# briandaniel/ParallelNonlinearOptimizationLibrary

Hardware: AMD Instinct MI355X
Metric: LM iters/sec at m=16384,n=2048 (higher is better)
Workload: dtype f64

## Files before the change

### parallelnonlinearoptimizationlibrary_amd/csrc/kernels/blas.hip

```cpp
#include "../pnol_internal.hpp"
#include "../pnol_comm.hpp"
#include "../pnol_env.hpp"

#include <cstdlib>

namespace pnol {
namespace {

constexpr int kWave = 64;

__device__ __forceinline__ double wave_sum(double v) {
#pragma unroll
    for (int m = 32; m >= 1; m >>= 1) v += __shfl_xor(v, m, kWave);
    return v;
}

constexpr int kU = 4;

template <int R>
__device__ __forceinline__ void gemv_load(double2 (&a)[R][kU], double2 (&xr)[kU], const double2* const (&arow)[R],
                                          const double2* __restrict__ xv, int base, int lane) {
#pragma unroll
    for (int u = 0; u < kU; ++u) xr[u] = xv[base + u * kWave + lane];
#pragma unroll
// ... 173 lines not shown
    __syncthreads();
    if (threadIdx.x < R && row0 + threadIdx.x < rows) {
        const int r = threadIdx.x;
        y[row0 + r] = -((part[0][r] + part[1][r]) + (part[2][r] + part[3][r]));
    }
}

template <int R, bool NT>
__global__ __launch_bounds__(256) void k_gemv_neg_wg(const double* __restrict__ A, long lda, int rows, int cols,
                                                     const double* __restrict__ x, double* __restrict__ y) {
    gemv_neg_wg_body<R, NT>(A, lda, rows, cols, x, y);
}

template <int R, bool VEC, bool XV>
__global__ __launch_bounds__(256) void k_gemv_neg_slices(const double* __restrict__ A, long lda, long sstride, int rows,
                                                         int m, int mS, int s0, const double* __restrict__ x,
                                                         double* __restrict__ y) {
    const int s = s0 + blockIdx.y;
    const int cols = max(0, min(mS, m - s * mS));
    gemv_neg_wg_body<R, true, VEC, XV>(A + (long)s * sstride, lda, rows, cols, x + (long)s * mS,
                                       y + (long)blockIdx.y * rows);
}

__global__ __launch_bounds__(256) void k_gemv_neg_scalar(const double* __restrict__ A, long lda, int rows, int cols,
                                                         const double* __restrict__ x, double* __restrict__ y) {
    const int lane = threadIdx.x & 63;
    const long row = (long)blockIdx.x * 4 + (threadIdx.x >> 6);
    if (row >= rows) return;
    const double* a = A + row * lda;
    double acc[4] = {0.0, 0.0, 0.0, 0.0};
    int c = lane;
    for (; c + 3 * kWave < cols; c += 4 * kWave)
// ... 302 lines not shown
#undef PNOL_GEMV_WG
        return launch_check();
    }
    int R = forced == 1 || forced == 2 || forced == 4 ? forced : (rows >= 8192 ? 2 : 1);
    const int blocks = (rows + 4 * R - 1) / (4 * R);
    if (R == 4)
        hipLaunchKernelGGL((k_gemv_neg<4>), dim3(blocks), dim3(256), 0, ctx->stream, A, (long)lda, rows, cols, x, y);
    else if (R == 2)
        hipLaunchKernelGGL((k_gemv_neg<2>), dim3(blocks), dim3(256), 0, ctx->stream, A, (long)lda, rows, cols, x, y);
    else
        hipLaunchKernelGGL((k_gemv_neg<1>), dim3(blocks), dim3(256), 0, ctx->stream, A, (long)lda, rows, cols, x, y);
    return launch_check();
}

int launch_gemv_neg_slices(pnol_ctx* ctx, const double* A, int lda, long sstride, int rows, int m, int mS, int s0,
                           int nsl, const double* x, double* y, hipStream_t stream) {
    if (!stream) stream = ctx->stream;
    if (!A || !x || !y || rows <= 0 || nsl <= 0 || (mS & 1)) return PNOL_ERR_ARG;
    static const int R = [] {
        const int v = env_atoi("PNOL_JTR_ROWS", 2);
        return (v == 1 || v == 4) ? v : 2;
    }();
    const bool vec = !((lda & 1) || (sstride & 1) || !aligned16(A));
    const bool xvec = aligned16(x);
    const dim3 grid((rows + R - 1) / R, nsl);
#define PNOL_SLICES(RR, V, XV)                                                                                      \
    hipLaunchKernelGGL((k_gemv_neg_slices<RR, V, XV>), grid, dim3(256), 0, stream, A, (long)lda, sstride, rows, m, mS, \
                       s0, x, y)
#define PNOL_SLICES_R(V, XV) \
    do { if (R == 1) PNOL_SLICES(1, V, XV); else if (R == 4) PNOL_SLICES(4, V, XV); else PNOL_SLICES(2, V, XV); } while (0)
    if (vec && xvec) PNOL_SLICES_R(true, true);
    else if (xvec) PNOL_SLICES_R(false, true);
    else if (vec) PNOL_SLICES_R(true, false);
    else PNOL_SLICES_R(false, false);
#undef PNOL_SLICES_R
#undef PNOL_SLICES
    return launch_check();
}

int launch_gemv_neg_seq(pnol_ctx* ctx, const double* A, int lda, int rows, int cols, const double* x, double* y) {
    if (!A || !x || !y || rows <= 0 || cols <= 0 || lda < cols) return PNOL_ERR_ARG;
    int blocks = (rows + 63) / 64;
    hipLaunchKernelGGL(k_gemv_neg_seq, dim3(blocks), dim3(64), 0, ctx->stream, A, (long)lda, rows, cols, x, y);
// ... 128 lines not shown
```

### parallelnonlinearoptimizationlibrary_amd/csrc/kernels/chol.hip

```cpp
#include "../pnol_internal.hpp"
#include "../pnol_comm.hpp"
#include "../chol_tasks.hpp"
#include "../pnol_env.hpp"

#include <algorithm>
#include <cstdlib>
#include <type_traits>

namespace pnol {
namespace {

constexpr int NB = 64;
constexpr int kPad = 18;
constexpr int kSub = NB * kPad;
constexpr int kStage = 4 * kSub;
constexpr int kSpin = 1 << 24;
constexpr int kInfoTimeout = kCholTimeout;
typedef double d4 __attribute__((ext_vector_type(4)));

__device__ __forceinline__ double readlane_d(double v, int lane) {
    const int lo = __builtin_amdgcn_readlane(__double2loint(v), lane);
    const int hi = __builtin_amdgcn_readlane(__double2hiint(v), lane);
    return __hiloint2double(hi, lo);
}
// ... 1802 lines not shown
    CholWs w;
    const bool persist = chol_persistent(variant) && (n + NB - 1) / NB >= 2;
    PNOL_CHECK(chol_ws(ctx, n, persist, w));
    const int T = w.T, N = w.N;
    for (int k = -1; k <= (persist ? -1 : T - 2); ++k) {
        const int R = T - 1 - k;
        const int grid = k < 0 ? 2 + std::min(N, 1024) : R + R * (R + 1) / 2;
        const int epoch = ++ctx->chol4_epoch;
        hipLaunchKernelGGL(k_chol_step, dim3(grid), dim3(256), 0, ctx->stream, w.P, w.Lm, w.ldp, T, k, w.W, w.bv, w.zv,
                           w.rowflag, epoch, dinfo, A, (long)lda, n, rhs, w.pf, persist ? w.npf : 0);
    }
    if (persist) PNOL_CHECK(chol_persist_launch(ctx, ctx->stream, w, dinfo, RedArgs{}));
    return chol_bwd_launch(ctx, ctx->stream, w, n, sigma, dinfo, xbase, xnext, xnext != nullptr);
}

__global__ __launch_bounds__(256) void k_chol_reducing_prep(double* __restrict__ P, long ldp, int T, int n,
                                                            double* __restrict__ bv, int* __restrict__ pflags,
                                                            int npflags, int* __restrict__ info, int vinit,
                                                            int* __restrict__ zc, int nz) {
    const int N = T * NB, tid = blockIdx.x * blockDim.x + threadIdx.x, nth = gridDim.x * blockDim.x;
    const int b0 = 2 * T, v1 = 3 * T + T * T;
    for (int q = tid; q < npflags; q += nth) pflags[q] = (q >= b0 && q < v1) ? vinit : 0;
    for (int q = tid; q < nz; q += nth) zc[q] = 0;
    for (int r = n + tid; r < N; r += nth) bv[r] = 0.0;
    if (n < N) {
        const long pad = (long)(N - n) * N + (long)n * (N - n);
        for (long e = tid; e < pad; e += nth) {
            int r, c;
            if (e < (long)(N - n) * N) {
                r = n + (int)(e / N);
                c = (int)(e % N);
            } else {
                const long f = e - (long)(N - n) * N;
                r = (int)(f / (N - n));
                c = n + (int)(f % (N - n));
            }
            P[(long)r * ldp + c] = r == c ? 1.0 : 0.0;
        }
    }
    if (tid == 0) *info = 0;
}

int launch_chol_reducing_prep(pnol_ctx* ctx, int n, int* dinfo, CholRed& cr) {
    if (!dinfo || n <= NB) return PNOL_ERR_ARG;
    cr.n = n;
    cr.dinfo = dinfo;
    return chol_ws(ctx, n, true, cr.w);
}

int launch_chol_reducing_start(pnol_ctx* ctx, const CholRed& cr, bool preloaded, int* zc, int nz) {
    const CholWs& w = cr.w;
    const int n = cr.n;
    const long pad = (long)(w.N - n) * w.N + (long)n * (w.N - n), work = std::max<long>(pad, w.npf);
    hipLaunchKernelGGL(k_chol_reducing_prep, dim3((unsigned)std::max<long>(1, std::min<long>(1024, (work + 255) / 256))),
                       dim3(256), 0, ctx->stream, w.P, w.ldp, w.T, n, w.bv, w.pf, w.npf, cr.dinfo, preloaded ? 0 : -1,
                       zc, zc ? nz : 0);
    return launch_check();
}

static int chol_red_run(pnol_ctx* ctx, hipStream_t st, const CholRed& cr, const RedArgs& red, double* sigma,
                        const double* xbase, double* xnext) {
    PNOL_CHECK(chol_persist_launch(ctx, st, cr.w, cr.dinfo, red));
    return chol_bwd_launch(ctx, st, cr.w, cr.n, sigma, cr.dinfo, xbase, xnext, true);
}

int launch_chol_preloaded_run(pnol_ctx* ctx, hipStream_t st, const CholRed& cr, double* sigma, const double* xbase,
                              double* xnext) {
    if (!sigma) return PNOL_ERR_ARG;
    RedArgs red;
    red.n = cr.n;
    red.preloaded = true;
// ... 33 lines not shown
```

### parallelnonlinearoptimizationlibrary_amd/csrc/kernels/syrk.hip

```cpp
#include "../pnol_internal.hpp"
#include "../pnol_comm.hpp"
#include "../pnol_env.hpp"

#include <algorithm>
#include <type_traits>
#include <vector>

namespace pnol {
namespace {

typedef double d4 __attribute__((ext_vector_type(4)));

constexpr int kPad = 18;

__device__ __forceinline__ unsigned diag_blocks(int w) {
    constexpr unsigned T[8] = {
        56u | 57u << 6 | 58u << 12 | 59u << 18 | 60u << 24 | 1u << 30,
        48u | 49u << 6 | 50u << 12 | 51u << 18 | 52u << 24 | 1u << 30,
        40u | 41u << 6 | 42u << 12 | 43u << 18 | 44u << 24 | 1u << 30,
        32u | 33u << 6 | 34u << 12 | 35u << 18 | 36u << 24 | 1u << 30,
        61u | 62u << 6 | 63u << 12 | 0u << 18,
        53u | 54u << 6 | 8u << 12 | 9u << 18,
        45u | 16u << 6 | 17u << 12 | 18u << 18,
        24u | 25u << 6 | 26u << 12 | 27u << 18};
// ... 52 lines not shown
#pragma unroll
    for (int q = 0; q < NV; ++q) *reinterpret_cast<double2*>(dst + 2 * q) = s.v[q];
}

#ifdef PNOL_SYRK_TIMELINE
__device__ unsigned long long g_syrk_tl[3 * 65536];
#endif

template <bool NTS, bool SC1 = false>
__device__ __forceinline__ void part_store(double v, double* p) {
    if constexpr (SC1) __hip_atomic_store(p, v, __ATOMIC_RELAXED, __HIP_MEMORY_SCOPE_AGENT);
    else if constexpr (NTS) __builtin_nontemporal_store(v, p);
    else *p = v;
}

template <int MODE, int TILE, int NW = 4, bool NTS = true, bool SC1 = false, bool DLAST = false>
__device__ __forceinline__ int syrk_tile_body(const double* __restrict__ X, long ldx, int nr, int K, int split_k,
                                              int kfirst, int kchunk, int sub, int slice0, int mS, long sstride,
                                              double* __restrict__ part, int tile0, int bid, int nblk,
                                              double (&lds)[2][2][TILE * kPad]) {
    constexpr int NT = 64 * NW, WC = NW / 2;
    constexpr int WTM = TILE / 2, WTN = TILE / WC, NBM = WTM / 16, NBN = WTN / 16;
#ifdef PNOL_SYRK_TIMELINE
    const unsigned long long tl0 = __builtin_amdgcn_s_memrealtime();
#endif
    int blk, t, sidx;
    {
        const int ntl = nblk / split_k, nsl = split_k / sub;
        const int u0 = bid / (ntl * nsl), rest = bid % (ntl * nsl);
        int tl = rest / nsl;
        if (DLAST) {
            const int nt = (int)((sqrt(8.0 * ntl + 1.0) - 1.0) * 0.5 + 0.5);
            const int noff = ntl - nt;
            if (tl < noff) {
                int r = (int)((sqrt(8.0 * tl + 1.0) + 1.0) * 0.5);
                while (r * (r - 1) / 2 > tl) --r;
                while ((r + 1) * r / 2 <= tl) ++r;
                tl = r * (r + 1) / 2 + (tl - r * (r - 1) / 2);
            } else {
                const int d = tl - noff;
                tl = d * (d + 1) / 2 + d;
            }
        }
        sidx = (rest % nsl) * sub + u0;
        blk = tl * split_k + sidx;
        t = tile0 + tl;
    }
    int ti, tj;
    tile_of(t, ti, tj);
    const bool diag = ti == tj;
    const int prow0 = ti * TILE, qrow0 = tj * TILE;
    const int slice = slice0 + sidx / sub, u = sidx % sub;
    X += (long)slice * (sstride - mS);
    const int kbeg = slice * mS + (u == 0 ? 0 : kfirst + (u - 1) * kchunk);
    const int kend = min(K, min((slice + 1) * mS, u == 0 ? slice * mS + kfirst : kbeg + kchunk));
    const int nstages = kend > kbeg ? (kend - kbeg + kTK - 1) / kTK : 0;

    const int lane = threadIdx.x & 63;
    const int wave = threadIdx.x >> 6;
    const int wr = wave / WC, wc = wave % WC;
    const bool ldx_even = (ldx & 1) == 0;

// ... 124 lines not shown
#pragma unroll
                for (int ni = 0; ni < NBN; ++ni)
#pragma unroll
                    for (int r = 0; r < 4; ++r) {
                        int row = wr * WTM + mi * 16 + orow + 4 * r;
                        int col = wc * WTN + ni * 16 + ocol;
                        part_store<NTS, SC1>(acc[mi][ni][r], out + row * ld + col);
                    }
        }
    }
#ifdef PNOL_SYRK_TIMELINE
    if (threadIdx.x == 0) {
        const unsigned long long tl1 = __builtin_amdgcn_s_memrealtime();
        const unsigned hw = __builtin_amdgcn_s_getreg(4 | (0 << 6) | (31 << 11));
        const unsigned xcc = __builtin_amdgcn_s_getreg(20 | (0 << 6) | (3 << 11));
        g_syrk_tl[3 * bid] = tl0;
        g_syrk_tl[3 * bid + 1] = tl1;
        g_syrk_tl[3 * bid + 2] = ((unsigned long long)xcc << 32) | hw;
    }
#endif
    return t;
}

template <int MODE, int TILE, int NW = 4, bool NTS = true>
__global__ __launch_bounds__(64 * NW, 2) void k_syrk_tile(const double* __restrict__ X, long ldx, int nr, int K,
                                                      int split_k, int kfirst, int kchunk, int sub, int slice0,
                                                      int mS, long sstride, double* __restrict__ part, int tile0) {
    __shared__ __attribute__((aligned(16))) double lds[2][2][TILE * kPad];
    (void)syrk_tile_body<MODE, TILE, NW, NTS>(X, ldx, nr, K, split_k, kfirst, kchunk, sub, slice0, mS, sstride, part,
                                              tile0, blockIdx.x, gridDim.x, lds);
}

constexpr int kS = kLmSlices;
static_assert(kS == 8, "tree8 spells out the 8-leaf tree");

__device__ __forceinline__ void tree_merge(double (&v)[kS], int (&sz)[kS]) {
#pragma unroll
    for (int w = 1; w < kS; w *= 2)
#pragma unroll
        for (int i = 0; i < kS; i += 2 * w)
            if (sz[i] == w && sz[i + w] == w) {
                v[i] = v[i] + v[i + w];
                sz[i] = 2 * w;
                sz[i + w] = 0;
            }
// ... 154 lines not shown
}

template <int SUB, int SR = 32>
__global__ __launch_bounds__(256) void k_syrk_reduce(const double* __restrict__ part, int ntiles, int sub_rt, int n,
                                                     double lambda, double* __restrict__ A, long lda,
                                                     double* __restrict__ diag_out, int tile0,
                                                     const double* __restrict__ jp = nullptr,
                                                     double* __restrict__ rhs = nullptr,
                                                     double* __restrict__ rhs2 = nullptr) {
    __shared__ double st[SR][kTile + 1];
    syrk_reduce_body<SUB, SR, 256>(part, ntiles, sub_rt, n, lambda, A, lda, diag_out, tile0, jp, rhs, rhs2, blockIdx.x,
                                   blockIdx.y, gridDim.x, st);
}

constexpr int kRedSR = 32, kRedSpin = 1 << 22;
template <int SUB, bool SC1, bool DLAST = false>
__global__ __launch_bounds__(512, 2) void k_syrk_red(const double* __restrict__ X, long ldx, int nr, int K,
                                                     int split_k, int kfirst, int kchunk, int sub, int mS, long sstride,
                                                     double* __restrict__ part, int nsyrk, int* __restrict__ tcnt,
                                                     int ntiles, int n, double lambda, double* __restrict__ A, long lda,
                                                     const double* __restrict__ jp, double* __restrict__ rhs,
                                                     double* __restrict__ rhs2, int* __restrict__ info) {
    __shared__ __attribute__((aligned(16))) double lds[2][2][kTile * kPad];
    __shared__ int ok_sh;
    const int b = blockIdx.x;
    if (b < nsyrk) {
        const int t = syrk_tile_body<0, kTile, 8, false, SC1, DLAST>(X, ldx, nr, K, split_k, kfirst, kchunk, sub, 0, mS,
                                                                    sstride, part, 0, b, nsyrk, lds);
        asm volatile("s_waitcnt vmcnt(0)" ::: "memory");
        __syncthreads();
        if (threadIdx.x == 0) {
            if constexpr (!SC1) {
                __builtin_amdgcn_fence(__ATOMIC_RELEASE, "agent");
                asm volatile("s_waitcnt vmcnt(0)" ::: "memory");
            }
            __hip_atomic_fetch_add(tcnt + t, 1, __ATOMIC_RELAXED, __HIP_MEMORY_SCOPE_AGENT);
        }
        return;
    }
    constexpr int NBX = kTile / kRedSR;
    const int r = b - nsyrk, bx = r % NBX, by = r / NBX;
    if (by < ntiles) {
        if (threadIdx.x == 0) {
            int it = 0, ok = 1;
            while (__hip_atomic_load(tcnt + by, __ATOMIC_RELAXED, __HIP_MEMORY_SCOPE_AGENT) < split_k) {
                __builtin_amdgcn_s_sleep(2);
                if (++it > kRedSpin) {
                    ok = 0;
                    atomicCAS(info, 0, kCholTimeout);
                    break;
                }
            }
            if (ok) {
                __builtin_amdgcn_fence(__ATOMIC_ACQUIRE, "agent");
                asm volatile("s_waitcnt vmcnt(0)" ::: "memory");
            }
            ok_sh = ok;
        }
        __syncthreads();
        if (!ok_sh) return;
    }
#ifdef PNOL_SYRK_TIMELINE
    const unsigned long long rt0 = __builtin_amdgcn_s_memrealtime();
#endif
    double(*st)[kTile + 1] = reinterpret_cast<double(*)[kTile + 1]>(&lds[0][0][0]);
    syrk_reduce_body<SUB, kRedSR, 512>(part, ntiles, sub, n, lambda, A, lda, nullptr, 0, jp, rhs, rhs2, bx, by, NBX, st);
#ifdef PNOL_SYRK_TIMELINE
    if (threadIdx.x == 0) {
        g_syrk_tl[3 * b] = rt0;
        g_syrk_tl[3 * b + 1] = __builtin_amdgcn_s_memrealtime();
        g_syrk_tl[3 * b + 2] = (unsigned long long)__builtin_amdgcn_s_getreg(20 | (0 << 6) | (3 << 11)) << 32;
    }
#endif
}
static_assert(kRedSR * (kTile + 1) <= 2 * 2 * kTile * kPad, "the reduce strip fits the SYRK's LDS");

__global__ void k_jtj_seq(const double* __restrict__ JT, long ldjt, int m, int n, double lambda,
                          double* __restrict__ A, long lda, double* __restrict__ diag_out) {
    int i = blockIdx.y * blockDim.y + threadIdx.y;
    int j = blockIdx.x * blockDim.x + threadIdx.x;
    if (i >= n || j >= n) return;
    const double* a = JT + (long)i * ldjt;
    const double* b = JT + (long)j * ldjt;
    double s = 0.0;
    for (int k = 0; k < m; ++k) s = s + a[k] * b[k];
    if (i == j) {
// ... 23 lines not shown
}
static int packed_ws(pnol_ctx* ctx, const LmNormalPlan& pl, double** packed) {
    return ws_get(ctx, "lm_packed", sizeof(double) * pl.packed_elems(), (void**)packed);
}

static void launch_reduce(hipStream_t st, const LmNormalPlan& pl, const double* part, int tile0, int ntl, double lambda,
                          double* A, long lda, double* jtj_diag, const double* jp = nullptr, double* rhs = nullptr,
                          double* bv = nullptr) {
    const int sub = pl.sc.sub;
    const auto k = sub == 1 ? k_syrk_reduce<1, 16> : sub == 2 ? k_syrk_reduce<2, 16> : sub == 4 ? k_syrk_reduce<4, 16>
                                                                                               : k_syrk_reduce<0, 16>;
    hipLaunchKernelGGL(k, dim3(kTile / 16, ntl + (jp ? 1 : 0)), dim3(256), 0, st, part, ntl, sub, pl.n, lambda, A, lda,
                       jtj_diag, tile0, jp, rhs, bv);
}

using SyrkRedKernel = decltype(&k_syrk_red<0, false, false>);
static SyrkRedKernel syrk_red_kernel(int sub, bool sc1, bool dlast) {
    if (sub != 2) return sc1 ? k_syrk_red<0, true, false> : k_syrk_red<0, false, false>;
    if (dlast) return sc1 ? k_syrk_red<2, true, true> : k_syrk_red<2, false, true>;
    return sc1 ? k_syrk_red<2, true, false> : k_syrk_red<2, false, false>;
}

static int launch_unpack(pnol_ctx* ctx, const LmNormalPlan& pl, const double* packed, long slot, double lambda,
                         double* A, long lda, double* jtj_diag) {
    hipLaunchKernelGGL(k_syrk_unpack, dim3(8, pl.ntiles), dim3(256), 0, ctx->stream, packed, pl.ntiles, pl.n, lambda,
                       slot, pl.tpr, A, lda, jtj_diag);
    return launch_check();
}

template <typename F>
static TreeNodes tree_table(const LmNormalPlan& pl, F ptr_of) {
    TreeNodes tn{};
    for (int c = 0; c < pl.NC; ++c) {
        tn.w[pl.node_lo[c]] = pl.node_w[c];
        tn.p[pl.node_lo[c]] = ptr_of(c);
// ... 5 lines not shown
static bool syrk_t64(bool sliced) { return env_atoi("PNOL_SYRK_T64", sliced) != 0; }

static void syrk_partials(pnol_ctx* ctx, hipStream_t stream, bool rows_variant, const double* X, long ldx,
                          long sstride, const LmNormalPlan& pl, int slice0, int nsl, int tile0, int ntl, double* part,
                          bool t64 = false) {
    const SliceCfg& sc = pl.sc;
    const int nr = pl.n, K = pl.m, split = nsl * sc.sub;
    LaunchTimer tm(ctx, rows_variant ? "syrk_rows" : "syrk");
    const auto k = t64 ? k_syrk_tile<4, 64> : rows_variant ? k_syrk_tile<2, 128, 8> : k_syrk_tile<0, 128, 8, false>;
    hipExtLaunchKernelGGL(k, dim3((t64 ? pl.ntiles64 : ntl) * split), dim3(t64 ? 256 : 512), 0, stream, tm.start(),
                          tm.stop(), 0, X, ldx, nr, K, split, sc.kfirst, sc.kchunk, sc.sub, slice0, sc.mS, sstride, part,
                          t64 ? 0 : tile0);
}

static int jtr_gemv(pnol_ctx* ctx, const LmNormalPlan& pl, const double* JT, int ldjt, long sstride, const double* F,
                    double** jp_out = nullptr) {
    if (!F) return PNOL_ERR_ARG;
    double* jp = nullptr;
    PNOL_CHECK(jtr_ws(ctx, pl, &jp));
    if (jp_out) *jp_out = jp;
    return launch_gemv_neg_slices(ctx, JT, ldjt, sstride, pl.n, pl.m, pl.sc.mS, pl.s0, pl.nsl(), F, jp);
}

static int jtr_tree(pnol_ctx* ctx, const LmNormalPlan& pl, double* out) {
    double* jp = nullptr;
    PNOL_CHECK(jtr_ws(ctx, pl, &jp));
    hipLaunchKernelGGL(k_tree_nodes, dim3((pl.n + 255) / 256, 1), dim3(256), 0, ctx->stream, (const double*)jp, 0L,
                       (long)pl.n, 1, pl.s0, pl.s1, pl.n, out, (long)pl.n, 0L);
    return launch_check();
}

int launch_jtj(pnol_ctx* ctx, const double* JT, int ldjt, int m, int n, double lambda, double* A, int lda,
               double* jtj_diag, const double* F, double* rhs) {
    if (!JT || !A || m <= 0 || n <= 0 || ldjt < m || lda < n) return PNOL_ERR_ARG;
    if (n <= PNOL_SEQ_MAX && m <= 4096) {
        dim3 blk(16, 16), grd((n + 15) / 16, (n + 15) / 16);
// ... 84 lines not shown
    if (n <= PNOL_SEQ_MAX) return PNOL_ERR_ARG;
    const LmNormalPlan pl = plan_for(m, n);
    const SliceCfg& sc = pl.sc;
    const int ntiles = pl.ntiles;
    const bool tasks = env_equals("PNOL_LM_REDUCE", "tasks");
    const bool tail = env_equals("PNOL_LM_REDUCE", "tail", true) && !syrk_t64(false);
    double *part = nullptr, *jp = nullptr;
    PNOL_CHECK(part_ws(ctx, pl.part_elems(), &part));
    PNOL_CHECK(jtr_ws(ctx, pl, &jp));
    void* tcnt = nullptr;
    if (tail) PNOL_CHECK(ws_get(ctx, "syrk_tcnt", sizeof(int) * (size_t)ntiles, &tcnt));
    CholRed cr;
    PNOL_CHECK(launch_chol_reducing_prep(ctx, n, dinfo, cr));
    if (fd_queued) PNOL_CHECK(lm_fd_commit(ctx, o, x));
    else PNOL_CHECK(launch_fd_jacobian(ctx, o, x, h, 0, n, F0, compute_f0, JT, ldjt));
    PNOL_CHECK(jtr_gemv(ctx, pl, JT, ldjt, sc.mS, F0));
    PNOL_CHECK(launch_chol_reducing_start(ctx, cr, !tasks, (int*)tcnt, ntiles));
    if (tail) {
        const int nsyrk = ntiles * pl.split, nred = (kTile / kRedSR) * (ntiles + 1);
        const bool sc1 = env_atoi("PNOL_SYRK_RED_SC1", 0) != 0;
        const bool dlast = env_default_on("PNOL_SYRK_DLAST");
        LaunchTimer tm(ctx, "syrk");
        hipExtLaunchKernelGGL(syrk_red_kernel(sc.sub, sc1, dlast), dim3(nsyrk + nred), dim3(512), 0, ctx->stream,
                              tm.start(), tm.stop(), 0, JT, (long)ldjt, n, m, pl.split, sc.kfirst, sc.kchunk, sc.sub,
                              sc.mS, (long)sc.mS, part, nsyrk, (int*)tcnt, ntiles, n, lambda, cr.w.P, cr.w.ldp,
                              (const double*)jp, rhs, cr.w.bv, cr.dinfo);
        PNOL_CHECK(launch_check());
    } else {
        syrk_partials(ctx, ctx->stream, false, JT, ldjt, sc.mS, pl, 0, kS, 0, ntiles, part, syrk_t64(false));
        PNOL_CHECK(launch_check());
        if (!tasks) {
            ScopedTimer tm(ctx, "syrk_reduce");
            launch_reduce(ctx->stream, pl, part, 0, ntiles, lambda, cr.w.P, cr.w.ldp, nullptr, jp, rhs, cr.w.bv);
            PNOL_CHECK(launch_check());
        }
    }
    ScopedTimer tm(ctx, "solve");
    if (!tasks)
        PNOL_CHECK(launch_chol_preloaded_run(ctx, ctx->stream, cr, sigma, x, xnext));
    else
        PNOL_CHECK(launch_chol_reducing_run(ctx, ctx->stream, cr, part, sc.sub, jp, lambda, rhs, sigma, x, xnext));
// ... 170 lines not shown
```

### parallelnonlinearoptimizationlibrary_amd/csrc/pnol_internal.hpp

```cpp
#pragma once

#include <hip/hip_ext.h>
#include <hip/hip_runtime.h>

#include <atomic>
#include <cmath>
#include <cstddef>
#include <cstdio>
#include <functional>
#include <map>
#include <mutex>
#include <string>
#include <vector>

#include "lm_normal_plan.hpp"
#include "pnol_amd.h"

namespace pnol {

struct Workspace {
    std::map<std::string, std::pair<void*, size_t>> bufs;
};

}
// ... 62 lines not shown

struct CholWs {
    int T = 0, N = 0;
    long ldp = 0;
    double *P = nullptr, *Lm = nullptr, *W = nullptr, *bv = nullptr, *zv = nullptr, *xw = nullptr;
    int *rowflag = nullptr, *bwdflag = nullptr, *pf = nullptr;
    int npf = 0;
    bool gran = false;
};
struct CholRed {
    CholWs w;
    int n = 0;
    int* dinfo = nullptr;
};

struct pnol_dobj {
    int kind = 0;
    int n = 0;
    int m = 0;
    double power = 2.0;
    double* p0 = nullptr;
    double* p1 = nullptr;
    double* p2 = nullptr;
    double* at = nullptr;
    size_t len0 = 0, len1 = 0;
    pnol_ctx* ctx = nullptr;
    int device = 0;
    unsigned long long id = pnol_dobj_next_id();
  private:
    static unsigned long long pnol_dobj_next_id() {
// ... 63 lines not shown
    hipError_t e = hipGetLastError();
    if (e != hipSuccess) {
        std::fprintf(stderr, "[pnol_amd] kernel launch failed: %s\n", hipGetErrorString(e));
        return PNOL_ERR_HIP;
    }
    return PNOL_OK;
}

constexpr int kCholTimeout = -7;
__host__ __device__ inline int solve_status_code(int info) { return info == 0 ? 0 : info == kCholTimeout ? 1 : 2; }
int launch_status_agree(pnol_ctx* ctx, int* dinfo);

int launch_gemv_neg(pnol_ctx* ctx, const double* A, int lda, int rows, int cols, const double* x, double* y);
int launch_gemv_neg_seq(pnol_ctx* ctx, const double* A, int lda, int rows, int cols, const double* x, double* y);
int launch_gemv_neg_slices(pnol_ctx* ctx, const double* A, int lda, long sstride, int rows, int m, int mS, int s0,
                           int nsl, const double* x, double* y, hipStream_t stream = nullptr);
int launch_bfgs_update_exact(pnol_ctx* ctx, double* D, int ldd, const double* y, const double* s, int n);
int launch_bfgs_pass(pnol_ctx* ctx, double* D, int ldd, int n, const double* s_p, const double* a_p,
                     const double* b_p, int write_back, const double* y, const double* g, double* u, double* w,
                     double* v, int rb = 0, int re = -1, int (*pw_gather)(pnol_ctx*, double*, int, int) = nullptr,
                     int ident_src = 0, const double* id_scale = nullptr);
int launch_set_identity(pnol_ctx* ctx, double* D, int ldd, int n, const double* scale, int rb = 0, int re = -1);
int launch_add(pnol_ctx* ctx, const double* x, const double* y, double* z, int n);
int launch_gather_sub(pnol_ctx* ctx, const double* D, int ldd, int n, const int* idx, int nsub, double* Dsub,
                      int lds);
int launch_gather_rows(pnol_ctx* ctx, const double* D, int ldd, const int* ridx, int nrows, int rbase, const int* cidx,
                       int ncols, double* Dsub, int lds);

int launch_jtj(pnol_ctx* ctx, const double* JT, int ldjt, int m, int n, double lambda, double* A, int lda,
               double* jtj_diag, const double* F = nullptr, double* rhs = nullptr);
int launch_fd_normal_solve(pnol_ctx* ctx, pnol_dobj* o, const double* x, const double* h, double* F0, int compute_f0,
// ... 5 lines not shown
int lm_fd_commit(pnol_ctx* ctx, pnol_dobj* o, const double* x);
int launch_jtj_from_partials(pnol_ctx* ctx, int m, int n, double lambda, double* A, int lda);
int launch_jtj_sharded(pnol_ctx* ctx, const double* JT, int ldjt, int m, int n, double lambda, double* A, int lda,
                       double* jtj_diag);
int launch_jtr(pnol_ctx* ctx, const double* JT, int ldjt, int m, int n, const double* F, double* rhs);

int launch_matrix_inverse(pnol_ctx* ctx, const double* B, int ldb, int n, double* Binv, int ldi, int* info_host);
int launch_chol_solve(pnol_ctx* ctx, const double* A, int lda, const double* rhs, double* sigma, int n, int* dinfo,
                      const double* xbase = nullptr, double* xnext = nullptr);
int launch_chol_solve_v(pnol_ctx* ctx, const double* A, int lda, const double* rhs, double* sigma, int n, int* dinfo,
                        int variant, const double* xbase = nullptr, double* xnext = nullptr);
int launch_solve(pnol_ctx* ctx, double* A, int lda, const double* rhs, double* sigma, int n, int method,
                 int* info);
int launch_chol_reducing_prep(pnol_ctx* ctx, int n, int* dinfo, CholRed& cr);
int launch_chol_reducing_start(pnol_ctx* ctx, const CholRed& cr, bool preloaded = false, int* zc = nullptr, int nz = 0);
int launch_chol_preloaded_run(pnol_ctx* ctx, hipStream_t st, const CholRed& cr, double* sigma, const double* xbase,
                              double* xnext);
int launch_chol_reducing_run(pnol_ctx* ctx, hipStream_t st, const CholRed& cr, const double* part, int sub,
                             const double* jp, double lambda, double* rhs, double* sigma, const double* xbase,
                             double* xnext);
int launch_chol_reducing_run_packed(pnol_ctx* ctx, hipStream_t st, const CholRed& cr, const double* packed, long slot,
                                    int tpr, const double* rhs, double lambda, double* sigma, const double* xbase,
                                    double* xnext);
int launch_lm_normal_solve(pnol_ctx* ctx, const double* JTs, int m, int n, double lambda, const double* F, double* rhs,
                           double* sigma, int* dinfo, const double* xbase, double* xnext);
int launch_lm_normal_unpack(pnol_ctx* ctx, int m, int n, double lambda, double* A, int lda);

int launch_dobj_eval(pnol_ctx* ctx, pnol_dobj* o, const double* x, double* out);
int launch_dobj_eval_ckpt(pnol_ctx* ctx, pnol_dobj* o, const double* x, double* out, int r0 = 0, int r1 = -1);
int launch_eval_batch(pnol_ctx* ctx, pnol_dobj* o, const double* Xs, int npts, double* out);
// ... 90 lines not shown
```

Before: 327.4.

## Fuse Cholesky prep into JTr GEMV and schedule SYRK via interleaved worklist

Moves the reducing-Cholesky workspace prep (padding, flag and counter init) into an extra grid row of the sliced JTr GEMV kernel, which removes a separate launch. Replaces the fixed SYRK-then-reduce block ordering with a worklist that interleaves whole tiles, split quarter-tiles and reduction strips. Reducers can then start on finished tiles while other SYRK tiles are still computing. This adds index-decoding cost per block and more complex completion counting (parts-based targets), which could cause load imbalance or spinning.

```diff
diff --git a/parallelnonlinearoptimizationlibrary_amd/csrc/kernels/blas.hip b/parallelnonlinearoptimizationlibrary_amd/csrc/kernels/blas.hip
--- a/parallelnonlinearoptimizationlibrary_amd/csrc/kernels/blas.hip
+++ b/parallelnonlinearoptimizationlibrary_amd/csrc/kernels/blas.hip
@@ -1,6 +1,7 @@
 #include "../pnol_internal.hpp"
 #include "../pnol_comm.hpp"
 #include "../pnol_env.hpp"
+#include "chol_prep.hpp"
 
 #include <cstdlib>
 
@@ -211,8 +212,12 @@
 
 template <int R, bool VEC, bool XV>
 __global__ __launch_bounds__(256) void k_gemv_neg_slices(const double* __restrict__ A, long lda, long sstride, int rows,
-                                                         int m, int mS, int s0, const double* __restrict__ x,
-                                                         double* __restrict__ y) {
+                                                         int m, int mS, int s0, int nsl, const double* __restrict__ x,
+                                                         double* __restrict__ y, const CholPrepArgs prep) {
+    if ((int)blockIdx.y >= nsl) {
+        chol_reducing_prep_body(prep, blockIdx.x * blockDim.x + threadIdx.x, gridDim.x * blockDim.x);
+        return;
+    }
     const int s = s0 + blockIdx.y;
     const int cols = max(0, min(mS, m - s * mS));
     gemv_neg_wg_body<R, true, VEC, XV>(A + (long)s * sstride, lda, rows, cols, x + (long)s * mS,
@@ -545,8 +550,9 @@
 }
 
 int launch_gemv_neg_slices(pnol_ctx* ctx, const double* A, int lda, long sstride, int rows, int m, int mS, int s0,
-                           int nsl, const double* x, double* y, hipStream_t stream) {
+                           int nsl, const double* x, double* y, hipStream_t stream, const CholPrepArgs* prep) {
     if (!stream) stream = ctx->stream;
+    const CholPrepArgs pa = prep ? *prep : CholPrepArgs{};
     if (!A || !x || !y || rows <= 0 || nsl <= 0 || (mS & 1)) return PNOL_ERR_ARG;
     static const int R = [] {
         const int v = env_atoi("PNOL_JTR_ROWS", 2);
@@ -554,10 +560,10 @@
     }();
     const bool vec = !((lda & 1) || (sstride & 1) || !aligned16(A));
     const bool xvec = aligned16(x);
-    const dim3 grid((rows + R - 1) / R, nsl);
+    const dim3 grid((rows + R - 1) / R, nsl + (prep ? 1 : 0));
 #define PNOL_SLICES(RR, V, XV)                                                                                      \
     hipLaunchKernelGGL((k_gemv_neg_slices<RR, V, XV>), grid, dim3(256), 0, stream, A, (long)lda, sstride, rows, m, mS, \
-                       s0, x, y)
+                       s0, nsl, x, y, pa)
 #define PNOL_SLICES_R(V, XV) \
     do { if (R == 1) PNOL_SLICES(1, V, XV); else if (R == 4) PNOL_SLICES(4, V, XV); else PNOL_SLICES(2, V, XV); } while (0)
     if (vec && xvec) PNOL_SLICES_R(true, true);
diff --git a/parallelnonlinearoptimizationlibrary_amd/csrc/kernels/chol.hip b/parallelnonlinearoptimizationlibrary_amd/csrc/kernels/chol.hip
--- a/parallelnonlinearoptimizationlibrary_amd/csrc/kernels/chol.hip
+++ b/parallelnonlinearoptimizationlibrary_amd/csrc/kernels/chol.hip
@@ -2,6 +2,7 @@
 #include "../pnol_comm.hpp"
 #include "../chol_tasks.hpp"
 #include "../pnol_env.hpp"
+#include "chol_prep.hpp"
 
 #include <algorithm>
 #include <cstdlib>
@@ -1840,31 +1841,8 @@
     return chol_bwd_launch(ctx, ctx->stream, w, n, sigma, dinfo, xbase, xnext, xnext != nullptr);
 }
 
-__global__ __launch_bounds__(256) void k_chol_reducing_prep(double* __restrict__ P, long ldp, int T, int n,
-                                                            double* __restrict__ bv, int* __restrict__ pflags,
-                                                            int npflags, int* __restrict__ info, int vinit,
-                                                            int* __restrict__ zc, int nz) {
-    const int N = T * NB, tid = blockIdx.x * blockDim.x + threadIdx.x, nth = gridDim.x * blockDim.x;
-    const int b0 = 2 * T, v1 = 3 * T + T * T;
-    for (int q = tid; q < npflags; q += nth) pflags[q] = (q >= b0 && q < v1) ? vinit : 0;
-    for (int q = tid; q < nz; q += nth) zc[q] = 0;
-    for (int r = n + tid; r < N; r += nth) bv[r] = 0.0;
-    if (n < N) {
-        const long pad = (long)(N - n) * N + (long)n * (N - n);
-        for (long e = tid; e < pad; e += nth) {
-            int r, c;
-            if (e < (long)(N - n) * N) {
-                r = n + (int)(e / N);
-                c = (int)(e % N);
-            } else {
-                const long f = e - (long)(N - n) * N;
-                r = (int)(f / (N - n));
-                c = n + (int)(f % (N - n));
-            }
-            P[(long)r * ldp + c] = r == c ? 1.0 : 0.0;
-        }
-    }
-    if (tid == 0) *info = 0;
+__global__ __launch_bounds__(256) void k_chol_reducing_prep(const CholPrepArgs a) {
+    chol_reducing_prep_body(a, blockIdx.x * blockDim.x + threadIdx.x, gridDim.x * blockDim.x);
 }
 
 int launch_chol_reducing_prep(pnol_ctx* ctx, int n, int* dinfo, CholRed& cr) {
@@ -1874,13 +1852,20 @@
     return chol_ws(ctx, n, true, cr.w);
 }
 
+CholPrepArgs chol_reducing_prep_args(const CholRed& cr, bool preloaded, int* zc, int nz) {
+    const CholWs& w = cr.w;
+    CholPrepArgs a;
+    a.P = w.P, a.ldp = w.ldp, a.T = w.T, a.N = w.T * NB, a.n = cr.n, a.bv = w.bv, a.pflags = w.pf, a.npflags = w.npf;
+    a.info = cr.dinfo, a.vinit = preloaded ? 0 : -1, a.zc = zc, a.nz = zc ? nz : 0;
+    return a;
+}
+
 int launch_chol_reducing_start(pnol_ctx* ctx, const CholRed& cr, bool preloaded, int* zc, int nz) {
     const CholWs& w = cr.w;
     const int n = cr.n;
     const long pad = (long)(w.N - n) * w.N + (long)n * (w.N - n), work = std::max<long>(pad, w.npf);
     hipLaunchKernelGGL(k_chol_reducing_prep, dim3((unsigned)std::max<long>(1, std::min<long>(1024, (work + 255) / 256))),
-                       dim3(256), 0, ctx->stream, w.P, w.ldp, w.T, n, w.bv, w.pf, w.npf, cr.dinfo, preloaded ? 0 : -1,
-                       zc, zc ? nz : 0);
+                       dim3(256), 0, ctx->stream, chol_reducing_prep_args(cr, preloaded, zc, nz));
     return launch_check();
 }
 
diff --git a/parallelnonlinearoptimizationlibrary_amd/csrc/kernels/chol_prep.hpp b/parallelnonlinearoptimizationlibrary_amd/csrc/kernels/chol_prep.hpp
--- /dev/null
+++ b/parallelnonlinearoptimizationlibrary_amd/csrc/kernels/chol_prep.hpp
@@ -0,0 +1,30 @@
+#pragma once
+#include "../pnol_internal.hpp"
+
+namespace pnol {
+
+__device__ __forceinline__ void chol_reducing_prep_body(const CholPrepArgs& a, int tid, int nth) {
+    const int T = a.T, N = a.N, n = a.n;
+    const int b0 = 2 * T, v1 = 3 * T + T * T;
+    for (int q = tid; q < a.npflags; q += nth) a.pflags[q] = (q >= b0 && q < v1) ? a.vinit : 0;
+    for (int q = tid; q < a.nz; q += nth) a.zc[q] = 0;
+    for (int r = n + tid; r < N; r += nth) a.bv[r] = 0.0;
+    if (n < N) {
+        const long pad = (long)(N - n) * N + (long)n * (N - n);
+        for (long e = tid; e < pad; e += nth) {
+            int r, c;
+            if (e < (long)(N - n) * N) {
+                r = n + (int)(e / N);
+                c = (int)(e % N);
+            } else {
+                const long f = e - (long)(N - n) * N;
+                r = (int)(f / (N - n));
+                c = n + (int)(f % (N - n));
+            }
+            a.P[(long)r * a.ldp + c] = r == c ? 1.0 : 0.0;
+        }
+    }
+    if (tid == 0) *a.info = 0;
+}
+
+}
diff --git a/parallelnonlinearoptimizationlibrary_amd/csrc/kernels/syrk.hip b/parallelnonlinearoptimizationlibrary_amd/csrc/kernels/syrk.hip
--- a/parallelnonlinearoptimizationlibrary_amd/csrc/kernels/syrk.hip
+++ b/parallelnonlinearoptimizationlibrary_amd/csrc/kernels/syrk.hip
@@ -1,6 +1,7 @@
 #include "../pnol_internal.hpp"
 #include "../pnol_comm.hpp"
 #include "../pnol_env.hpp"
+#include "../syrk_worklist.hpp"
 
 #include <algorithm>
 #include <type_traits>
@@ -90,38 +91,26 @@
     else *p = v;
 }
 
-template <int MODE, int TILE, int NW = 4, bool NTS = true, bool SC1 = false, bool DLAST = false>
-__device__ __forceinline__ int syrk_tile_body(const double* __restrict__ X, long ldx, int nr, int K, int split_k,
-                                              int kfirst, int kchunk, int sub, int slice0, int mS, long sstride,
-                                              double* __restrict__ part, int tile0, int bid, int nblk,
-                                              double (&lds)[2][2][TILE * kPad]) {
+__device__ __forceinline__ void syrk_unit_of(int bid, int nblk, int split_k, int sub, int tile0, int& blk, int& t,
+                                             int& sidx) {
+    const int ntl = nblk / split_k, nsl = split_k / sub;
+    const int u0 = bid / (ntl * nsl), rest = bid % (ntl * nsl);
+    const int tl = rest / nsl;
+    sidx = (rest % nsl) * sub + u0;
+    blk = tl * split_k + sidx;
+    t = tile0 + tl;
+}
+
+template <int MODE, int TILE, int NW = 4, bool NTS = true, bool SC1 = false>
+__device__ __forceinline__ void syrk_tile_body(const double* __restrict__ X, long ldx, int nr, int K, int split_k,
+                                               int kfirst, int kchunk, int sub, int slice0, int mS, long sstride,
+                                               double* __restrict__ part, int t, int sidx, int blk, int tlid,
+                                               double (&lds)[2][2][TILE * kPad]) {
     constexpr int NT = 64 * NW, WC = NW / 2;
     constexpr int WTM = TILE / 2, WTN = TILE / WC, NBM = WTM / 16, NBN = WTN / 16;
 #ifdef PNOL_SYRK_TIMELINE
     const unsigned long long tl0 = __builtin_amdgcn_s_memrealtime();
 #endif
-    int blk, t, sidx;
-    {
-        const int ntl = nblk / split_k, nsl = split_k / sub;
-        const int u0 = bid / (ntl * nsl), rest = bid % (ntl * nsl);
-        int tl = rest / nsl;
-        if (DLAST) {
-            const int nt = (int)((sqrt(8.0 * ntl + 1.0) - 1.0) * 0.5 + 0.5);
-            const int noff = ntl - nt;
-            if (tl < noff) {
-                int r = (int)((sqrt(8.0 * tl + 1.0) + 1.0) * 0.5);
-                while (r * (r - 1) / 2 > tl) --r;
-                while ((r + 1) * r / 2 <= tl) ++r;
-                tl = r * (r + 1) / 2 + (tl - r * (r - 1) / 2);
-            } else {
-                const int d = tl - noff;
-                tl = d * (d + 1) / 2 + d;
-            }
-        }
-        sidx = (rest % nsl) * sub + u0;
-        blk = tl * split_k + sidx;
-        t = tile0 + tl;
-    }
     int ti, tj;
     tile_of(t, ti, tj);
     const bool diag = ti == tj;
@@ -276,12 +265,11 @@
         const unsigned long long tl1 = __builtin_amdgcn_s_memrealtime();
         const unsigned hw = __builtin_amdgcn_s_getreg(4 | (0 << 6) | (31 << 11));
         const unsigned xcc = __builtin_amdgcn_s_getreg(20 | (0 << 6) | (3 << 11));
-        g_syrk_tl[3 * bid] = tl0;
-        g_syrk_tl[3 * bid + 1] = tl1;
-        g_syrk_tl[3 * bid + 2] = ((unsigned long long)xcc << 32) | hw;
+        g_syrk_tl[3 * tlid] = tl0;
+        g_syrk_tl[3 * tlid + 1] = tl1;
+        g_syrk_tl[3 * tlid + 2] = ((unsigned long long)xcc << 32) | hw;
     }
 #endif
-    return t;
 }
 
 template <int MODE, int TILE, int NW = 4, bool NTS = true>
@@ -289,8 +277,10 @@
                                                       int split_k, int kfirst, int kchunk, int sub, int slice0,
                                                       int mS, long sstride, double* __restrict__ part, int tile0) {
     __shared__ __attribute__((aligned(16))) double lds[2][2][TILE * kPad];
-    (void)syrk_tile_body<MODE, TILE, NW, NTS>(X, ldx, nr, K, split_k, kfirst, kchunk, sub, slice0, mS, sstride, part,
-                                              tile0, blockIdx.x, gridDim.x, lds);
+    int blk, t, sidx;
+    syrk_unit_of(blockIdx.x, gridDim.x, split_k, sub, tile0, blk, t, sidx);
+    syrk_tile_body<MODE, TILE, NW, NTS>(X, ldx, nr, K, split_k, kfirst, kchunk, sub, slice0, mS, sstride, part, t, sidx,
+                                        blk, blockIdx.x, lds);
 }
 
 constexpr int kS = kLmSlices;
@@ -475,19 +465,31 @@
 }
 
 constexpr int kRedSR = 32, kRedSpin = 1 << 22;
-template <int SUB, bool SC1, bool DLAST = false>
+static_assert(kTile / kRedSR == kSyrkStrips, "syrk_worklist.hpp counts the strips of a tile");
+template <int SUB, bool SC1>
 __global__ __launch_bounds__(512, 2) void k_syrk_red(const double* __restrict__ X, long ldx, int nr, int K,
                                                      int split_k, int kfirst, int kchunk, int sub, int mS, long sstride,
-                                                     double* __restrict__ part, int nsyrk, int* __restrict__ tcnt,
-                                                     int ntiles, int n, double lambda, double* __restrict__ A, long lda,
-                                                     const double* __restrict__ jp, double* __restrict__ rhs,
-                                                     double* __restrict__ rhs2, int* __restrict__ info) {
+                                                     double* __restrict__ part, const SyrkWorklist wl,
+                                                     int* __restrict__ tcnt, int ntiles, int n, double lambda,
+                                                     double* __restrict__ A, long lda, const double* __restrict__ jp,
+                                                     double* __restrict__ rhs, double* __restrict__ rhs2,
+                                                     int* __restrict__ info) {
     __shared__ __attribute__((aligned(16))) double lds[2][2][kTile * kPad];
     __shared__ int ok_sh;
     const int b = blockIdx.x;
-    if (b < nsyrk) {
-        const int t = syrk_tile_body<0, kTile, 8, false, SC1, DLAST>(X, ldx, nr, K, split_k, kfirst, kchunk, sub, 0, mS,
-                                                                    sstride, part, 0, b, nsyrk, lds);
+    const SyrkItem it = syrk_item(wl, b);
+    if (it.kind == kSyrkWhole || it.kind == kSyrkPart) {
+        if (it.kind == kSyrkWhole) {
+            syrk_tile_body<0, kTile, 8, false, SC1>(X, ldx, nr, K, split_k, kfirst, kchunk, sub, 0, mS, sstride, part, it.t,
+                                                    it.sidx, it.t * split_k + it.sidx, b, lds);
+        } else {
+            int ti, tj;
+            tile_of(it.t, ti, tj);
+            const int ti64 = 2 * ti + (it.q >> 1), tj64 = 2 * tj + (it.q & 1);
+            syrk_tile_body<4, kTile / 2, 8, false, SC1>(X, ldx, nr, K, split_k, kfirst, kchunk, sub, 0, mS, sstride, part,
+                                                        ti64 * (ti64 + 1) / 2 + tj64, it.sidx, 0, b,
+                                                        reinterpret_cast<double(&)[2][2][kTile / 2 * kPad]>(lds));
+        }
         asm volatile("s_waitcnt vmcnt(0)" ::: "memory");
         __syncthreads();
         if (threadIdx.x == 0) {
@@ -495,18 +497,23 @@
                 __builtin_amdgcn_fence(__ATOMIC_RELEASE, "agent");
                 asm volatile("s_waitcnt vmcnt(0)" ::: "memory");
             }
-            __hip_atomic_fetch_add(tcnt + t, 1, __ATOMIC_RELAXED, __HIP_MEMORY_SCOPE_AGENT);
+            __hip_atomic_fetch_add(tcnt + it.t, it.kind == kSyrkWhole ? kSyrkParts : 1, __ATOMIC_RELAXED,
+                                   __HIP_MEMORY_SCOPE_AGENT);
         }
         return;
     }
     constexpr int NBX = kTile / kRedSR;
-    const int r = b - nsyrk, bx = r % NBX, by = r / NBX;
+    const int bx = it.q, by = it.t;
+#ifdef PNOL_SYRK_TIMELINE
+    const unsigned long long rt0 = __builtin_amdgcn_s_memrealtime();
+#endif
     if (by < ntiles) {
         if (threadIdx.x == 0) {
-            int it = 0, ok = 1;
-            while (__hip_atomic_load(tcnt + by, __ATOMIC_RELAXED, __HIP_MEMORY_SCOPE_AGENT) < split_k) {
+            int spin = 0, ok = 1;
+            const int target = wl.target();
+            while (__hip_atomic_load(tcnt + by, __ATOMIC_RELAXED, __HIP_MEMORY_SCOPE_AGENT) < target) {
                 __builtin_amdgcn_s_sleep(2);
-                if (++it > kRedSpin) {
+                if (++spin > kRedSpin) {
                     ok = 0;
                     atomicCAS(info, 0, kCholTimeout);
                     break;
@@ -522,7 +529,7 @@
         if (!ok_sh) return;
     }
 #ifdef PNOL_SYRK_TIMELINE
-    const unsigned long long rt0 = __builtin_amdgcn_s_memrealtime();
+    const unsigned long long rt1 = __builtin_amdgcn_s_memrealtime();
 #endif
     double(*st)[kTile + 1] = reinterpret_cast<double(*)[kTile + 1]>(&lds[0][0][0]);
     syrk_reduce_body<SUB, kRedSR, 512>(part, ntiles, sub, n, lambda, A, lda, nullptr, 0, jp, rhs, rhs2, bx, by, NBX, st);
@@ -530,7 +537,8 @@
     if (threadIdx.x == 0) {
         g_syrk_tl[3 * b] = rt0;
         g_syrk_tl[3 * b + 1] = __builtin_amdgcn_s_memrealtime();
-        g_syrk_tl[3 * b + 2] = (unsigned long long)__builtin_amdgcn_s_getreg(20 | (0 << 6) | (3 << 11)) << 32;
+        g_syrk_tl[3 * b + 2] = (unsigned long long)__builtin_amdgcn_s_getreg(20 | (0 << 6) | (3 << 11)) << 32 |
+                               ((rt1 - rt0) & 0xffffffffull);
     }
 #endif
 }
@@ -584,11 +592,16 @@
                        jtj_diag, tile0, jp, rhs, bv);
 }
 
-using SyrkRedKernel = decltype(&k_syrk_red<0, false, false>);
-static SyrkRedKernel syrk_red_kernel(int sub, bool sc1, bool dlast) {
-    if (sub != 2) return sc1 ? k_syrk_red<0, true, false> : k_syrk_red<0, false, false>;
-    if (dlast) return sc1 ? k_syrk_red<2, true, true> : k_syrk_red<2, false, true>;
-    return sc1 ? k_syrk_red<2, true, false> : k_syrk_red<2, false, false>;
+using SyrkRedKernel = decltype(&k_syrk_red<0, false>);
+static SyrkRedKernel syrk_red_kernel(int sub, bool sc1) {
+    if (sub != 2) return sc1 ? k_syrk_red<0, true> : k_syrk_red<0, false>;
+    return sc1 ? k_syrk_red<2, true> : k_syrk_red<2, false>;
+}
+
+static SyrkWorklist syrk_worklist_for(const LmNormalPlan& pl) {
+    const bool dlast = env_default_on("PNOL_SYRK_DLAST") && pl.sc.sub == 2;
+    return syrk_worklist(pl.nt, pl.split / pl.sc.sub, pl.sc.sub, dlast, env_atoi("PNOL_SYRK_SPLIT", kSyrkSplitDefault),
+                         env_atoi("PNOL_SYRK_RED_LAG", kSyrkLagDefault));
 }
 
 static int launch_unpack(pnol_ctx* ctx, const LmNormalPlan& pl, const double* packed, long slot, double lambda,
@@ -624,12 +637,12 @@
 }
 
 static int jtr_gemv(pnol_ctx* ctx, const LmNormalPlan& pl, const double* JT, int ldjt, long sstride, const double* F,
-                    double** jp_out = nullptr) {
+                    double** jp_out = nullptr, const CholPrepArgs* prep = nullptr) {
     if (!F) return PNOL_ERR_ARG;
     double* jp = nullptr;
     PNOL_CHECK(jtr_ws(ctx, pl, &jp));
     if (jp_out) *jp_out = jp;
-    return launch_gemv_neg_slices(ctx, JT, ldjt, sstride, pl.n, pl.m, pl.sc.mS, pl.s0, pl.nsl(), F, jp);
+    return launch_gemv_neg_slices(ctx, JT, ldjt, sstride, pl.n, pl.m, pl.sc.mS, pl.s0, pl.nsl(), F, jp, nullptr, prep);
 }
 
 static int jtr_tree(pnol_ctx* ctx, const LmNormalPlan& pl, double* out) {
@@ -744,17 +757,21 @@
     PNOL_CHECK(launch_chol_reducing_prep(ctx, n, dinfo, cr));
     if (fd_queued) PNOL_CHECK(lm_fd_commit(ctx, o, x));
     else PNOL_CHECK(launch_fd_jacobian(ctx, o, x, h, 0, n, F0, compute_f0, JT, ldjt));
-    PNOL_CHECK(jtr_gemv(ctx, pl, JT, ldjt, sc.mS, F0));
-    PNOL_CHECK(launch_chol_reducing_start(ctx, cr, !tasks, (int*)tcnt, ntiles));
     if (tail) {
-        const int nsyrk = ntiles * pl.split, nred = (kTile / kRedSR) * (ntiles + 1);
+        const CholPrepArgs prep = chol_reducing_prep_args(cr, true, (int*)tcnt, ntiles);
+        PNOL_CHECK(jtr_gemv(ctx, pl, JT, ldjt, sc.mS, F0, nullptr, &prep));
+    } else {
+        PNOL_CHECK(jtr_gemv(ctx, pl, JT, ldjt, sc.mS, F0));
+        PNOL_CHECK(launch_chol_reducing_start(ctx, cr, !tasks, (int*)tcnt, ntiles));
+    }
+    if (tail) {
         const bool sc1 = env_atoi("PNOL_SYRK_RED_SC1", 0) != 0;
-        const bool dlast = env_default_on("PNOL_SYRK_DLAST");
+        const SyrkWorklist wl = syrk_worklist_for(pl);
         LaunchTimer tm(ctx, "syrk");
-        hipExtLaunchKernelGGL(syrk_red_kernel(sc.sub, sc1, dlast), dim3(nsyrk + nred), dim3(512), 0, ctx->stream,
-                              tm.start(), tm.stop(), 0, JT, (long)ldjt, n, m, pl.split, sc.kfirst, sc.kchunk, sc.sub,
-                              sc.mS, (long)sc.mS, part, nsyrk, (int*)tcnt, ntiles, n, lambda, cr.w.P, cr.w.ldp,
-                              (const double*)jp, rhs, cr.w.bv, cr.dinfo);
+        hipExtLaunchKernelGGL(syrk_red_kernel(sc.sub, sc1), dim3(wl.grid()), dim3(512), 0, ctx->stream, tm.start(),
+                              tm.stop(), 0, JT, (long)ldjt, n, m, pl.split, sc.kfirst, sc.kchunk, sc.sub, sc.mS,
+                              (long)sc.mS, part, wl, (int*)tcnt, ntiles, n, lambda, cr.w.P, cr.w.ldp, (const double*)jp,
+                              rhs, cr.w.bv, cr.dinfo);
         PNOL_CHECK(launch_check());
     } else {
         syrk_partials(ctx, ctx->stream, false, JT, ldjt, sc.mS, pl, 0, kS, 0, ntiles, part, syrk_t64(false));
diff --git a/parallelnonlinearoptimizationlibrary_amd/csrc/pnol_internal.hpp b/parallelnonlinearoptimizationlibrary_amd/csrc/pnol_internal.hpp
--- a/parallelnonlinearoptimizationlibrary_amd/csrc/pnol_internal.hpp
+++ b/parallelnonlinearoptimizationlibrary_amd/csrc/pnol_internal.hpp
@@ -100,6 +100,19 @@
     int* dinfo = nullptr;
 };
 
+struct CholPrepArgs {
+    double* P = nullptr;
+    long ldp = 0;
+    int T = 0, N = 0, n = 0;
+    double* bv = nullptr;
+    int* pflags = nullptr;
+    int npflags = 0;
+    int* info = nullptr;
+    int vinit = 0;
+    int* zc = nullptr;
+    int nz = 0;
+};
+
 struct pnol_dobj {
     int kind = 0;
     int n = 0;
@@ -193,7 +206,8 @@
 int launch_gemv_neg(pnol_ctx* ctx, const double* A, int lda, int rows, int cols, const double* x, double* y);
 int launch_gemv_neg_seq(pnol_ctx* ctx, const double* A, int lda, int rows, int cols, const double* x, double* y);
 int launch_gemv_neg_slices(pnol_ctx* ctx, const double* A, int lda, long sstride, int rows, int m, int mS, int s0,
-                           int nsl, const double* x, double* y, hipStream_t stream = nullptr);
+                           int nsl, const double* x, double* y, hipStream_t stream = nullptr,
+                           const CholPrepArgs* prep = nullptr);
 int launch_bfgs_update_exact(pnol_ctx* ctx, double* D, int ldd, const double* y, const double* s, int n);
 int launch_bfgs_pass(pnol_ctx* ctx, double* D, int ldd, int n, const double* s_p, const double* a_p,
                      const double* b_p, int write_back, const double* y, const double* g, double* u, double* w,
@@ -229,6 +243,7 @@
                  int* info);
 int launch_chol_reducing_prep(pnol_ctx* ctx, int n, int* dinfo, CholRed& cr);
 int launch_chol_reducing_start(pnol_ctx* ctx, const CholRed& cr, bool preloaded = false, int* zc = nullptr, int nz = 0);
+CholPrepArgs chol_reducing_prep_args(const CholRed& cr, bool preloaded, int* zc, int nz);
 int launch_chol_preloaded_run(pnol_ctx* ctx, hipStream_t st, const CholRed& cr, double* sigma, const double* xbase,
                               double* xnext);
 int launch_chol_reducing_run(pnol_ctx* ctx, hipStream_t st, const CholRed& cr, const double* part, int sub,
diff --git a/parallelnonlinearoptimizationlibrary_amd/csrc/syrk_worklist.hpp b/parallelnonlinearoptimizationlibrary_amd/csrc/syrk_worklist.hpp
--- /dev/null
+++ b/parallelnonlinearoptimizationlibrary_amd/csrc/syrk_worklist.hpp
@@ -0,0 +1,138 @@
+#pragma once
+
+#include <cmath>
+
+#ifndef PNOL_HD
+#ifdef __HIPCC__
+#define PNOL_HD __host__ __device__
+#else
+#define PNOL_HD
+#endif
+#endif
+
+namespace pnol {
+
+constexpr int kSyrkParts = 4;
+constexpr int kSyrkStrips = 4;
+constexpr int kSyrkSplitDefault = 0;
+constexpr int kSyrkLagDefault = 1 << 30;
+
+enum SyrkItemKind { kSyrkWhole = 0, kSyrkPart = 1, kSyrkStrip = 2, kSyrkRhs = 3 };
+struct SyrkItem {
+    int kind;
+    int t;
+    int sidx;
+    int q;
+};
+
+struct SyrkWorklist {
+    int nt, ntiles, nsl, sub, dlast;
+    int noff;
+    int nsplit;
+    int q0;
+    int lag, oB;
+    int rB, tB;
+    int nA, nB, nC, nD;
+    PNOL_HD int grid() const { return nA + nB + nC + nD; }
+    PNOL_HD int syrk_items() const { return nA + nB - kSyrkStrips * oB + nC; }
+    PNOL_HD int target() const { return nsl * sub * kSyrkParts; }
+};
+
+PNOL_HD inline int syrk_tri_row(int t) {
+    int r = (int)((sqrt(8.0 * t + 1.0) - 1.0) * 0.5);
+    while ((r + 1) * (r + 2) / 2 <= t) ++r;
+    while (r * (r + 1) / 2 > t) --r;
+    return r;
+}
+PNOL_HD inline int syrk_off_tile(int k) {
+    const int ti = syrk_tri_row(k) + 1;
+    return ti * (ti + 1) / 2 + (k - ti * (ti - 1) / 2);
+}
+PNOL_HD inline int syrk_diag_tile(int d) { return d * (d + 1) / 2 + d; }
+
+PNOL_HD inline int syrk_order_tile(const SyrkWorklist& w, int o) {
+    if (!w.dlast) return o;
+    return o < w.noff ? syrk_off_tile(o) : syrk_diag_tile(o - w.noff);
+}
+PNOL_HD inline int syrk_off_before(const SyrkWorklist& w, int o) {
+    if (w.dlast) return o < w.noff ? o : w.noff;
+    return o >= w.ntiles ? w.noff : o - syrk_tri_row(o);
+}
+PNOL_HD inline int syrk_whole_before(const SyrkWorklist& w, int o) {
+    const int off = syrk_off_before(w, o), rank = off * w.nsl;
+    return (o - off) * w.nsl + (rank < w.q0 ? rank : w.q0);
+}
+PNOL_HD inline int syrk_b_pos(const SyrkWorklist& w, int o) {
+    int r = o - w.lag;
+    r = r < 0 ? 0 : r > w.oB ? w.oB : r;
+    return syrk_whole_before(w, o) + kSyrkStrips * r;
+}
+
+PNOL_HD inline SyrkWorklist syrk_worklist(int nt, int nsl, int sub, bool dlast, int split, int lag) {
+    SyrkWorklist w;
+    w.nt = nt, w.ntiles = nt * (nt + 1) / 2, w.nsl = nsl, w.sub = sub, w.dlast = dlast ? 1 : 0;
+    w.noff = w.ntiles - nt;
+    const int noffu = w.noff * nsl;
+    w.nsplit = sub < 2 || split <= 0 ? 0 : split < noffu ? split : noffu;
+    w.q0 = noffu - w.nsplit;
+    w.lag = lag < 0 ? 0 : lag > w.ntiles ? w.ntiles : lag;
+    int first_split = w.ntiles;
+    if (w.nsplit > 0) first_split = dlast ? w.q0 / nsl : syrk_off_tile(w.q0 / nsl);
+    w.oB = w.ntiles - w.lag < first_split ? w.ntiles - w.lag : first_split;
+    if (dlast && w.oB > w.noff) w.oB = w.noff;
+    if (dlast) {
+        w.rB = syrk_tri_row(w.oB) + 1;
+        w.tB = w.rB + w.oB;
+    } else {
+        w.rB = 0, w.tB = w.oB;
+    }
+    w.nA = (sub - 1) * w.ntiles * nsl;
+    w.nB = syrk_b_pos(w, w.ntiles);
+    w.nC = w.nsplit * kSyrkParts;
+    w.nD = kSyrkStrips * (w.ntiles - w.oB + 1);
+    return w;
+}
+
+PNOL_HD inline SyrkItem syrk_item(const SyrkWorklist& w, int b) {
+    SyrkItem it;
+    if (b < w.nA) {
+        const int per = w.ntiles * w.nsl, u = b / per, rest = b % per;
+        it.kind = kSyrkWhole, it.t = syrk_order_tile(w, rest / w.nsl), it.sidx = (rest % w.nsl) * w.sub + u, it.q = 0;
+        return it;
+    }
+    b -= w.nA;
+    if (b < w.nB) {
+        int lo = 0, hi = w.ntiles - 1;
+        while (lo < hi) {
+            const int mid = (lo + hi + 1) / 2;
+            if (syrk_b_pos(w, mid) <= b) lo = mid;
+            else hi = mid - 1;
+        }
+        const int local = b - syrk_b_pos(w, lo);
+        const int whole = syrk_whole_before(w, lo + 1) - syrk_whole_before(w, lo);
+        if (local < whole) {
+            it.kind = kSyrkWhole, it.t = syrk_order_tile(w, lo), it.sidx = local * w.sub + w.sub - 1, it.q = 0;
+        } else {
+            it.kind = kSyrkStrip, it.t = syrk_order_tile(w, lo - w.lag), it.sidx = 0, it.q = local - whole;
+        }
+        return it;
+    }
+    b -= w.nB;
+    if (b < w.nC) {
+        const int rank = w.q0 + b / kSyrkParts;
+        it.kind = kSyrkPart, it.t = syrk_off_tile(rank / w.nsl), it.sidx = (rank % w.nsl) * w.sub + w.sub - 1;
+        it.q = b % kSyrkParts;
+        return it;
+    }
+    b -= w.nC;
+    const int k = b / kSyrkStrips;
+    it.sidx = 0, it.q = b % kSyrkStrips;
+    if (k >= w.ntiles - w.oB) {
+        it.kind = kSyrkRhs, it.t = w.ntiles;
+    } else {
+        it.kind = kSyrkStrip, it.t = k < w.rB ? syrk_diag_tile(k) : w.tB + k - w.rB;
+    }
+    return it;
+}
+
+}
```

New measurement: 320.9. -2.0%, worse.
